# daviidsilvaa/MPI-Model

Measured on AMD Instinct MI355X. Metric: cell-updates/s (GCUPS) per step + % of HBM roofline, higher is better.
Workload: dtype f64; 1 GPU; c3: 32768x32768 fp64 global, row slabs (BASELINE configs[2]); ranks=1, rows_per_gpu=32768, n_attr=1, parallelism=row-slab x1, rows_per_wave=1656

## Files before the change

mpi-model_amd/csrc/mm_engine.hip:

```cpp
#include <rccl/rccl.h>

#include <algorithm>
#include <cmath>
#include <cstdio>
#include <cstdlib>
#include <cstring>
#include <map>
#include <string>
#include <vector>

#include "../../include/mpimodel.h"
#include "mm_inst.hpp"
#include "mm_plan.hpp"

static_assert(MM_FIELD_MAX_STEPS == mm::kFieldMaxSteps, "include/mpimodel.h: MM_FIELD_MAX_STEPS");

namespace {

thread_local std::string g_last_error;

int fail(int code, const std::string& msg) {
    g_last_error = msg;
    return code;
}
// ... 15 lines not shown
#define MM_TRY(expr)             \
    do {                         \
        int rc_ = (expr);        \
        if (rc_ != MM_OK) return rc_; \
    } while (0)

struct Transfer {
    int a, b;
    double rate;
};

struct Pass {
    std::vector<Transfer> pre, post;
    int diffuse_mask = 0;
    double drate[mm::kMaxAttr] = {0, 0, 0, 0};
    int field_mask = 0;
};

struct FlowDesc {
    int kind, a, b;
    double rate;
};

}

struct mm_engine {
    mm_desc d{};
    int na = 1;
    long long pitch = 0;
    long long rows_alloc = 0;
    double* base = nullptr;
    size_t bytes = 0;
    double* buf[2][mm::kMaxAttr] = {};
    int cur = 0;
    double* fld_base[mm::kMaxAttr] = {};
    double* fld[mm::kMaxAttr] = {};
    long long fld_rows[mm::kMaxAttr][2] = {};
    hipStream_t s_comp = nullptr, s_comm = nullptr;
    hipEvent_t ev_ready = nullptr, ev_halo = nullptr;
    hipEvent_t ev_comp_mark = nullptr, ev_comm_done = nullptr;
    bool comm_live = false;
    ncclComm_t comm = nullptr;

    std::vector<FlowDesc> flows;
    std::vector<Pass> passes;

    mm::PlanIn pin;
    int th_env = 8;
    std::map<const mm::KernelInst*, int> slots;
    bool self_halo = false;
    int variant = 0;
    double* partials = nullptr;
    long long partials_cap = 0;
    double* hist = nullptr;
    unsigned long long* hist_n = nullptr;
    long long hist_cap = 0;
    long long hist_host = 0;
    double* sum_tmp = nullptr;
    long long sum_blocks = 0;

    long long steps_done = 0;

    std::map<std::tuple<int, long long, long long, long long>, std::pair<hipGraphExec_t, int>> graphs;

    int graph_state = 0;
    long long graph_launches = 0;
    int graph_count = 0;
    std::string graph_note;

    bool timing = false;
    std::vector<hipEvent_t> ev_pool;
    std::vector<double> ev_bytes;
    size_t ev_used = 0;
    long long timed_launches = 0;
    double timed_ms = 0.0;
    double timed_bytes = 0.0;
};

namespace {

int set_device(mm_engine* e) {
    MM_HIP(hipSetDevice(e->d.device));
    return MM_OK;
}

void drop_graphs(mm_engine* e) {
    for (auto& kv : e->graphs) (void)hipGraphExecDestroy(kv.second.first);
    e->graphs.clear();
}

int compile_passes(mm_engine* e) {
    e->passes.clear();
    Pass cur;
    bool open = false;
    for (const FlowDesc& f : e->flows) {
        const bool fieldf = f.kind == MM_FLOW_DIFFUSE_FIELD;
        if (open && (fieldf ? (!cur.field_mask || (cur.field_mask & (1 << f.a))) : cur.field_mask != 0)) {
            e->passes.push_back(cur);
            open = false;
        }
        if (fieldf) {
            if (!open) {
                cur = Pass();
                open = true;
            }
            cur.field_mask |= 1 << f.a;
// ... 186 lines not shown
    return MM_OK;
}

int split_comm(mm_engine* e, int depth) {
    if (!e->comm_live) MM_HIP(hipStreamWaitEvent(e->s_comm, e->ev_comp_mark, 0));
    if (rccl_halo(e)) MM_TRY(halo_rccl(e, depth));
    MM_HIP(hipStreamWaitEvent(e->s_comm, e->ev_comp_mark, 0));
    return MM_OK;
}

int unsplit_halo(mm_engine* e, int depth) {
    if (!rccl_halo(e)) return MM_OK;
    MM_HIP(hipEventRecord(e->ev_ready, e->s_comp));
    MM_HIP(hipStreamWaitEvent(e->s_comm, e->ev_ready, 0));
    MM_TRY(halo_rccl(e, depth));
    MM_HIP(hipEventRecord(e->ev_halo, e->s_comm));
    MM_HIP(hipStreamWaitEvent(e->s_comp, e->ev_halo, 0));
    return MM_OK;
}

int launch(mm_engine* e, const mm::PassLaunches& pl, bool red, const mm::PassArgs& A, hipStream_t s,
           bool border) {
    const int nt = border ? 0 : e->variant;
    if (pl.kern.kernel != mm::kOneStep)
        MM_HIP(mm::launch_kstep(
            inst_key(e, pl.kern.kernel, pl.depth, pl.kern.cols, A.seg != 0, red, nt & 1), A, s));
    else if (A.field_mask)
        MM_HIP(mm::launch_field(e->na, red, A, s, nt));
    else
        MM_HIP(mm::launch_pass(e->na, red, A, s, e->variant));
    return MM_OK;
}

void set_launch(mm::PassArgs& A, const mm::Launch& l) {
    A.ra0 = (int)l.lo, A.ra1 = (int)l.hi, A.rb0 = (int)l.lo2, A.rb1 = (int)l.hi2;
    A.seg = l.seg, A.th = l.th, A.th_edge = l.th_edge, A.xcd_remap = l.xcd_remap;
    A.nstrips = l.nstrips;
    A.waves_a = l.waves_a, A.waves_total = l.waves_total, A.partial_base = l.partial_base;
    const mm::Wide6& w = l.c6;
    A.c6_top = w.top, A.c6_bot = w.bot, A.c6_col = w.col, A.c6_rcol = w.rcol;
    A.c6_strips = w.strips, A.c6_rstrips = w.rstrips, A.c6_th = w.th;
    A.c6_band0 = w.band0, A.c6_band1 = w.band1, A.c6_frame = w.frame;
}

int enqueue_pass(mm_engine* e, const Pass& p, int k, int mask, bool time_it, bool prime = false) {
    const bool red = mask != 0;
    const mm::PassLaunches pl = mm::pass_launches(e->pin, k, red);
    mm::PassArgs A;
    fill_args(e, p, A);
    const int perm = pl.kern.kernel == mm::kWide ? relabel(e, A) : kPermIdentity;
    mm::PassArgs B = A;
    set_launch(A, pl.interior);
    set_launch(B, pl.border);
    if (prime) {
        A.waves_total = B.waves_total = 0;
        A.waves_a = B.waves_a = -1;
        MM_TRY(launch(e, pl, red, A, e->s_comp, false));
        if (pl.split) MM_TRY(launch(e, pl, red, B, e->s_comm, true));
        return MM_OK;
    }
    if (pl.split)
        MM_TRY(split_comp(e));
    else if (e->pin.split)
        MM_TRY(unsplit_halo(e, pl.depth));
    hipEvent_t t0 = nullptr, t1 = nullptr;
    if (time_it) {
        t0 = next_event(e);
        t1 = next_event(e);
        if (!t0 || !t1) return fail(MM_ERR_HIP, "hipEventCreate failed");
        e->ev_bytes.resize(e->ev_used / 2);
        e->ev_bytes.back() = (16.0 * e->na + 8.0 * __builtin_popcount((unsigned)p.field_mask)) *
                             (double)(pl.interior.hi - pl.interior.lo) * (double)e->d.W;
        MM_HIP(hipEventRecord(t0, e->s_comp));
    }
    MM_TRY(launch(e, pl, red, A, e->s_comp, false));
    if (time_it) MM_HIP(hipEventRecord(t1, e->s_comp));
    if (pl.split) {
        MM_TRY(split_comm(e, pl.depth));
        MM_TRY(launch(e, pl, red, B, e->s_comm, true));
        MM_HIP(hipEventRecord(e->ev_comm_done, e->s_comm));
        e->comm_live = true;
        if (red) MM_HIP(hipStreamWaitEvent(e->s_comp, e->ev_comm_done, 0));
    }
    if (red && pl.kern.kernel == mm::kOneStep)
        MM_HIP(mm::launch_finalize(e->partials, pl.total, e->na, e->hist, e->hist_n, e->hist_cap,
                                   e->s_comp, 1));
    else if (red)
        MM_HIP(mm::launch_finalize_levels(e->partials, pl.total, k, e->na, mask, e->hist,
                                          e->hist_n, e->hist_cap, e->s_comp, perm));
    e->cur ^= 1;
    return MM_OK;
}

int enqueue_steps(mm_engine* e, long long first, long long n, long long reduce_every,
                  bool time_it) {
    long long s = first;
    const long long end = first + n;
    auto red = [&](long long step) { return reduce_every > 0 && step % reduce_every == 0; };
    if (mm::kstep_ok(e->pin)) {
        for (int k : mm::pass_lengths(e->pin, n)) {
            int mask = 0;
            for (int j = 0; j < k; ++j)
                if (red(s + j)) mask |= 1 << j;
            MM_TRY(enqueue_pass(e, e->passes[0], k, mask, time_it));
            s += k;
        }
    } else {
        const int np = (int)e->passes.size();
        for (; s < end; ++s)
            for (int pi = 0; pi < np; ++pi)
                MM_TRY(enqueue_pass(e, e->passes[pi], 1, red(s) && pi == np - 1, time_it));
    }
    if (e->comm_live) {
        MM_HIP(hipStreamWaitEvent(e->s_comp, e->ev_comm_done, 0));
        e->comm_live = false;
    }
    return MM_OK;
}

int agree_capture(mm_engine* e, bool ok) {
    if (!e->comm || e->d.nranks <= 1) return ok ? MM_OK : MM_ERR_HIP;
    int v = ok ? 1 : 0;
    int* dv = reinterpret_cast<int*>(e->sum_tmp);
    if (hipStreamSynchronize(e->s_comp) != hipSuccess ||
        hipStreamSynchronize(e->s_comm) != hipSuccess ||
        hipMemcpy(dv, &v, sizeof v, hipMemcpyHostToDevice) != hipSuccess ||
        ncclAllReduce(dv, dv, 1, ncclInt32, ncclMin, e->comm, e->s_comm) != ncclSuccess ||
// ... 176 lines not shown
        return fail(MM_ERR_INVALID, "mm_engine_create: a single slab must own the whole grid");
    if (d.halo_mode == MM_HALO_RCCL && !d.comm_id)
        return fail(MM_ERR_INVALID, "mm_engine_create: MM_HALO_RCCL needs comm_id");
    if (d.nranks > 1 && d.halo_mode == MM_HALO_NONE)
        return fail(MM_ERR_INVALID, "mm_engine_create: nranks > 1 needs a halo mode");
    if (d.W > (1LL << 30) || d.h > (1LL << 30))
        return fail(MM_ERR_INVALID, "mm_engine_create: slab too large");

    mm_engine* e = new mm_engine();
    e->d = d;
    e->na = d.n_attr;
    e->pitch = (d.W + mm::kStripCols - 1) / mm::kStripCols * mm::kStripCols;
    e->rows_alloc = d.h + 2 * mm::kGhost;
    mm::PlanIn& pin = e->pin;
    pin.H = d.H, pin.W = d.W, pin.h = d.h, pin.x_init = d.x_init, pin.nranks = d.nranks;
    pin.pitch = e->pitch, pin.n_attr = d.n_attr;
    pin.min_rows = std::min<long long>(d.h, d.H / d.nranks);
    pin.knobs = mm::read_knobs([](const char* name) -> const char* { return std::getenv(name); });
    e->th_env = pin.knobs.th;
    pin.slots = [e](mm::Kernel kernel, int k, bool red) { return slots_per_cu(e, kernel, k, red); };
    pin.slots6 = [e](int k) { return slots_per_cu(e, mm::kWide, k, false, mm::kWide6Cols); };
    e->variant = mm::kernel_variant(pin);

    auto cleanup = [&](int rc) {
        mm_engine_destroy(e);
        return rc;
    };
    hipError_t he = hipSetDevice(d.device);
    if (he != hipSuccess) return cleanup(fail(MM_ERR_HIP, std::string("hipSetDevice: ") + hipGetErrorString(he)));
    he = hipDeviceGetAttribute(&e->pin.ncu, hipDeviceAttributeMultiprocessorCount, d.device);
    if (he != hipSuccess || e->pin.ncu <= 0) e->pin.ncu = 256;

    const size_t per = (size_t)e->rows_alloc * (size_t)e->pitch;
    const size_t per_al = (per + 31) / 32 * 32;
    e->bytes = sizeof(double) * per_al * 2 * (size_t)e->na;
    if (hipStreamCreateWithFlags(&e->s_comp, hipStreamNonBlocking) != hipSuccess ||
        hipStreamCreateWithFlags(&e->s_comm, hipStreamNonBlocking) != hipSuccess ||
        hipEventCreateWithFlags(&e->ev_ready, hipEventDisableTiming) != hipSuccess ||
        hipEventCreateWithFlags(&e->ev_halo, hipEventDisableTiming) != hipSuccess ||
        hipEventCreateWithFlags(&e->ev_comp_mark, hipEventDisableTiming) != hipSuccess ||
        hipEventCreateWithFlags(&e->ev_comm_done, hipEventDisableTiming) != hipSuccess)
        return cleanup(fail(MM_ERR_HIP, "stream/event creation failed"));

    he = hipMalloc(&e->base, e->bytes);
    if (he != hipSuccess) return cleanup(fail(MM_ERR_NOMEM, std::string("hipMalloc: ") + hipGetErrorString(he)));
    he = hipMemsetAsync(e->base, 0, e->bytes, e->s_comp);
    if (he != hipSuccess) return cleanup(fail(MM_ERR_HIP, std::string("hipMemsetAsync: ") + hipGetErrorString(he)));
    for (int k = 0; k < 2; ++k)
        for (int a = 0; a < e->na; ++a)
            e->buf[k][a] = e->base + per_al * (size_t)(k * e->na + a) + mm::kGhost * e->pitch;

    int rc = ensure_partials(e);
    if (rc != MM_OK) return cleanup(rc);
    e->hist_cap = 1 << 12;
    if (hipMalloc(&e->hist, sizeof(double) * (size_t)e->hist_cap * e->na) != hipSuccess ||
        hipMalloc(&e->hist_n, 2 * sizeof(unsigned long long)) != hipSuccess ||
        hipMemsetAsync(e->hist_n, 0, 2 * sizeof(unsigned long long), e->s_comp) != hipSuccess)
        return cleanup(fail(MM_ERR_NOMEM, "history allocation failed"));
    e->sum_blocks = std::min<long long>(1024, std::max<long long>(1, d.h));
    if (hipMalloc(&e->sum_tmp, sizeof(double) * (size_t)(e->sum_blocks + mm::kMaxAttr)) != hipSuccess)
        return cleanup(fail(MM_ERR_NOMEM, "sum scratch allocation failed"));
    he = hipStreamSynchronize(e->s_comp);
    if (he != hipSuccess) return cleanup(fail(MM_ERR_HIP, std::string("hipStreamSynchronize: ") + hipGetErrorString(he)));

    e->self_halo = e->pin.knobs.self_halo && d.nranks == 1 && d.halo_mode == MM_HALO_RCCL;
    if ((d.nranks > 1 || e->self_halo) && d.halo_mode == MM_HALO_RCCL) {
        int v = 0;
        if (ncclGetVersion(&v) != ncclSuccess || v != NCCL_VERSION_CODE) {
            char msg[160];
            std::snprintf(msg, sizeof msg,
                          "RCCL %d loaded, engine built against %d: load libmpimodel_hip.so "
                          "before any library that bundles its own librccl (e.g. torch)",
                          v, NCCL_VERSION_CODE);
            return cleanup(fail(MM_ERR_RCCL, msg));
        }
        ncclUniqueId id;
        std::memcpy(&id, d.comm_id, sizeof id);
        ncclResult_t nr = ncclCommInitRank(&e->comm, d.nranks, id, d.rank);
        if (nr != ncclSuccess)
            return cleanup(fail(MM_ERR_RCCL, std::string("ncclCommInitRank: ") + ncclGetErrorString(nr)));
        long long hmin = d.h;
        double* dv = e->sum_tmp;
        if (hipMemcpy(dv, &hmin, sizeof hmin, hipMemcpyHostToDevice) != hipSuccess ||
            ncclAllReduce(dv, dv, 1, ncclInt64, ncclMin, e->comm, e->s_comm) != ncclSuccess ||
            hipStreamSynchronize(e->s_comm) != hipSuccess ||
            hipMemcpy(&hmin, dv, sizeof hmin, hipMemcpyDeviceToHost) != hipSuccess)
            return cleanup(fail(MM_ERR_RCCL, "min slab rows all-reduce failed"));
        e->pin.min_rows = hmin;
        e->pin.split = true;
    } else if (d.nranks > 1 && d.halo_mode == MM_HALO_HOST) {
        long long x0 = 0, hh = 0;
        if (mm_partition_rows(d.H, d.nranks, d.rank, &x0, &hh) != MM_OK || x0 != d.x_init ||
            hh != d.h)
            return cleanup(fail(MM_ERR_INVALID, "mm_engine_create: MM_HALO_HOST slabs must be "
                                                "mm_partition_rows(H, nranks, rank)"));
        e->pin.split = true;
    }
    *out = e;
    return MM_OK;
}

int mm_engine_destroy(mm_engine* e) {
    if (!e) return MM_OK;
    (void)hipSetDevice(e->d.device);
    if (e->s_comp) (void)hipStreamSynchronize(e->s_comp);
    if (e->s_comm) (void)hipStreamSynchronize(e->s_comm);
    drop_graphs(e);
    if (e->comm) (void)ncclCommDestroy(e->comm);
    for (hipEvent_t ev : e->ev_pool) (void)hipEventDestroy(ev);
    if (e->ev_ready) (void)hipEventDestroy(e->ev_ready);
    if (e->ev_halo) (void)hipEventDestroy(e->ev_halo);
    if (e->ev_comp_mark) (void)hipEventDestroy(e->ev_comp_mark);
    if (e->ev_comm_done) (void)hipEventDestroy(e->ev_comm_done);
    if (e->s_comp) (void)hipStreamDestroy(e->s_comp);
    if (e->s_comm) (void)hipStreamDestroy(e->s_comm);
    if (e->base) (void)hipFree(e->base);
    for (double* f : e->fld_base)
        if (f) (void)hipFree(f);
    if (e->partials) (void)hipFree(e->partials);
    if (e->hist) (void)hipFree(e->hist);
    if (e->hist_n) (void)hipFree(e->hist_n);
    if (e->sum_tmp) (void)hipFree(e->sum_tmp);
    (void)hipGetLastError();
    delete e;
    return MM_OK;
}

int mm_engine_info(mm_engine* e, mm_info* info) {
    if (!e || !info) return fail(MM_ERR_INVALID, "mm_engine_info: null");
    std::memset(info, 0, sizeof *info);
    info->pitch = e->pitch;
    info->bytes_device = (long long)e->bytes;
    info->n_passes = (int)e->passes.size();
    const mm::SlabPlan sp = mm::slab_plan(e->pin);
    info->kernel = sp.kernel;
    info->rows_per_wave = sp.rows_per_wave;
    info->waves_per_pass = sp.waves_per_pass;
    info->seg_waves_per_cu = sp.seg_waves_per_cu;
    if (sp.kernel == mm::kWide && e->na > 1)
        info->chain_kernel = (wring(e) && sp.steps_per_launch == 8) ? MM_CHAIN_RING : MM_CHAIN_RUNTIME;
    info->steps_done = e->steps_done;
    info->fused_attrs = e->na;
    info->steps_per_launch = info->halo_depth = sp.steps_per_launch;
    info->graph_state = e->graph_state;
    info->graph_count = e->graph_count;
    info->graph_launches = e->graph_launches;
    info->hist_entries = e->hist_host;
    std::snprintf(info->graph_note, sizeof info->graph_note, "%s", e->graph_note.c_str());
    return MM_OK;
}

int mm_fill(mm_engine* e, int attr, int mode, double value, unsigned long long seed) {
    if (!e || attr < 0 || attr >= e->na || (mode != MM_FILL_UNIFORM && mode != MM_FILL_RANDOM))
        return fail(MM_ERR_INVALID, "mm_fill: bad arguments");
    MM_TRY(set_device(e));
    MM_HIP(mm::launch_fill(e->buf[e->cur][attr], e->pitch, e->d.H, e->d.W, e->d.x_init, e->d.h,
                           mode, value, seed, e->s_comp));
    MM_HIP(hipStreamSynchronize(e->s_comp));
    e->steps_done = 0;
    return MM_OK;
}

int mm_upload(mm_engine* e, int attr, const double* host) {
    if (!e || !host || attr < 0 || attr >= e->na) return fail(MM_ERR_INVALID, "mm_upload: bad arguments");
    MM_TRY(set_device(e));
    MM_HIP(hipMemcpy2DAsync(e->buf[e->cur][attr], sizeof(double) * e->pitch, host,
                            sizeof(double) * e->d.W, sizeof(double) * e->d.W, e->d.h,
                            hipMemcpyHostToDevice, e->s_comp));
    MM_HIP(hipStreamSynchronize(e->s_comp));
    e->steps_done = 0;
    return MM_OK;
}
// ... 443 lines not shown
```

mpi-model_amd/csrc/mm_geom.hpp:

```cpp
#pragma once

namespace mm {

constexpr int kMaxAttr = 4;
constexpr int kMaxChain = 4;
constexpr int kStripCols = 128;
constexpr int kWavesPerBlock = 4;
constexpr int kBlock = 64 * kWavesPerBlock;
constexpr int kMaxSteps = 10;
constexpr int kMaxWide = 20;
constexpr int kGhost = kMaxWide;
constexpr int kBorderRows = 4;
constexpr int kSegPrefetch1 = 8;
constexpr int kWide20Waves = 4;
constexpr int kWideRingWaves = 4;
constexpr int kWide6Cols = 6;

constexpr int span3(long long n, long long i) {
    return (i >= 0 && i < n) ? 1 + (i > 0) + (i < n - 1) : 0;
}

inline int passk_out_cols(int k) { return kStripCols - 4 * ((k + 1) / 2); }

inline int passk_max_steps(int na) { return na == 1 ? kMaxSteps : 2; }

inline long long passk_max_rows(int k, long long pitch) {
    return (1LL << 31) / (pitch * 8) - (3 * k + 2 * kSegPrefetch1 + 8);
}

constexpr int kFieldMaxSteps = 4;
constexpr int kFieldPrefetch = 8;
constexpr int field_ring(int k) {
    return (kFieldPrefetch + 2 * (k - 1) + kFieldPrefetch - 1) / kFieldPrefetch * kFieldPrefetch;
}

inline long long fieldk_max_rows(int k, long long pitch) {
    return (1LL << 31) / (pitch * 8) - (3 * k + 2 * field_ring(k) + 8);
}

inline bool wide_has(int k, int c, int na) {
    if (na > 1) return na == 4 && c == 2 && (k == 4 || k == 8);
    return c == 4 && (k == 4 || k == 8 || k == 12 || k == 16 || k == 20);
}

inline int wide_out_cols(int k, int c) {
    return 64 * c - 2 * c * ((k + c - 1) / c);
}

struct Wide6Cols {
    int col, rcol, strips, rstrips;
};
inline Wide6Cols wide6_cols(long long W) {
    const int o4 = wide_out_cols(kMaxWide, 4), o6 = wide_out_cols(kMaxWide, kWide6Cols);
    const int halo = kWide6Cols * ((kMaxWide + kWide6Cols - 1) / kWide6Cols);
    const long long room = W - o4 - (halo + 1);
    const int n = room >= o6 && W < (1LL << 30) ? (int)(room / o6) : 0;
    const int rcol = o4 + n * o6;
    return {o4, rcol, n, n ? (int)((W - rcol + o4 - 1) / o4) : 0};
}

inline int wide_waves_per_block(int k, int c, int na, bool ring) {
    if (!wide_has(k, c, na)) return 0;
    if (na > 1 && k == 8 && ring) return kWideRingWaves;
    if (na == 1 && k == 20) return kWide20Waves;
    return 4;
}

}
```

mpi-model_amd/csrc/mm_internal.hpp:

```cpp
#pragma once

#include <hip/hip_runtime.h>

#include "mm_geom.hpp"

namespace mm {

struct PassArgs {
    const double* in[kMaxAttr];
    double* out[kMaxAttr];
    long long H, W, x_init, pitch;
    int ra0, ra1, rb0, rb1;
    int th;
    int nstrips;
    long long waves_a;
    long long waves_total;
    int diffuse_mask;
    int npre, npost;
    double drate[kMaxAttr];
    signed char pre_a[kMaxChain], pre_b[kMaxChain];
    signed char post_a[kMaxChain], post_b[kMaxChain];
    double pre_r[kMaxChain], post_r[kMaxChain];
    double* partials;
    long long partial_base;
    int xcd_remap;
    int seg;
    int th_edge;
    const double* field[kMaxAttr];
    int field_mask;
    int c6_top, c6_bot;
    int c6_col, c6_rcol;
    int c6_strips, c6_rstrips;
    int c6_th;
    long long c6_band0, c6_band1, c6_frame;
};

hipError_t launch_pass(int na, bool reduce, const PassArgs& a, hipStream_t s, int variant);
hipError_t launch_field(int na, bool reduce, const PassArgs& a, hipStream_t s, int variant);
hipError_t launch_finalize_levels(const double* partials, long long n, int k, int na, int mask,
                                  double* hist, unsigned long long* hist_n, long long cap,
                                  hipStream_t s, int perm);
hipError_t launch_fill(double* buf, long long pitch, long long H, long long W, long long x_init,
                       long long h, int mode, double value, unsigned long long seed, hipStream_t s);
hipError_t launch_point(double* buf, long long pitch, long long H, long long W, long long x_init,
                        long long h, long long sx, long long sy, double captured, double rate,
                        hipStream_t s);
hipError_t launch_finalize(const double* partials, long long n, int na, double* hist,
                           unsigned long long* hist_n, long long cap, hipStream_t s,
                           int entries = 1);
hipError_t launch_slab_sum(const double* buf, long long pitch, long long W, long long h,
                           double* partials, long long nblocks, double* out_sum, hipStream_t s);

}
```

mpi-model_amd/csrc/mm_plan.cpp:

```cpp
#include "mm_plan.hpp"

#include <algorithm>
#include <cmath>
#include <cstdlib>

namespace mm {

namespace {

constexpr double kAny = 1e300;

struct KnobRow {
    const char* name;
    char type;
    double lo, hi;
    void (*set)(Knobs&, double);
};

const KnobRow kKnobRows[] = {
    {"MM_GRAPH", 'i', -kAny, kAny, [](Knobs& k, double v) { k.graphs_ok = v != 0; }},
    {"MM_GRAPH_MIN_STEPS", 'i', 1, 256, [](Knobs& k, double v) { k.graph_min = (long long)v; }},
    {"MM_GRAPH_MAX_LAUNCHES", 'i', 1, 4096, [](Knobs& k, double v) { k.graph_max = (long long)v; }},
    {"MM_ROWS_PER_WAVE", 'i', 8, 32, [](Knobs& k, double v) { if (v == 8 || v == 16 || v == 32) k.th = (int)v; }},
    {"MM_FUSE", 'i', -kAny, kAny, [](Knobs& k, double v) { k.passk = k.passk && v != 0; }},
    {"MM_PASSK", 'i', -kAny, kAny, [](Knobs& k, double v) { k.passk = k.passk && v != 0; }},
    {"MM_WIDE", 'i', -kAny, kAny, [](Knobs& k, double v) { k.wide = v != 0 ? 1 : 0; }},
    {"MM_STEPS_PER_PASS", 'i', 1, kAny,
     [](Knobs& k, double d) {
         const int v = (int)std::min(d, 1e9);
         if (v <= kMaxSteps || (k.wide != 0 && (wide_has(v, 4, 1) || wide_has(v, 2, 4)))) k.kpass = v;
         k.kpass_multi = std::min(v, 2);
     }},
    {"MM_PASS_PLAN", 'i', -kAny, kAny, [](Knobs& k, double v) { k.plan = v != 0; }},
    {"MM_SEG_WAVES", 'd', 0, kAny, [](Knobs& k, double v) { k.seg_waves = v; }},
    {"MM_SEG_EDGE", 'd', 0, 1, [](Knobs& k, double v) { k.seg_edge = v; }},
    {"MM_XCD_REMAP", 'i', -kAny, kAny, [](Knobs& k, double v) { k.xcd = v != 0; }},
    {"MM_BORDER_SEGMENTS", 'i', -kAny, kAny, [](Knobs& k, double v) { k.border_segments = v != 0; }},
    {"MM_CHAIN_RING", 'i', -kAny, kAny, [](Knobs& k, double v) { k.ring_ok = v != 0; }},
    {"MM_SYNC_SPIN", 'i', -kAny, kAny, [](Knobs& k, double v) { k.sync_spin = v != 0; }},
    {"MM_SELF_HALO", 'i', -kAny, kAny, [](Knobs& k, double v) { k.self_halo = v != 0; }},
    {"MM_KERNEL_VARIANT", 'i', 0, kAny, [](Knobs& k, double v) { k.variant = (int)std::min(v, 1e9); }},
    {"MM_FIELD_STEPS", 'i', 0, kFieldMaxSteps, [](Knobs& k, double v) { k.field_steps = (int)v; }},
    {"MM_FIELD_HALO", 'i', 1, kFieldMaxSteps, [](Knobs& k, double v) { k.field_halo = (int)v; }},
    {"MM_WIDE_COLS", 'i', 4, kWide6Cols, [](Knobs& k, double v) { if (v != 5) k.wide_cols = (int)v; }},
};

}

Knobs read_knobs(const std::function<const char*(const char*)>& get) {
    Knobs k;
    for (const KnobRow& r : kKnobRows) {
        const char* s = get(r.name);
        if (!s) continue;
        const double v = r.type == 'i' ? (double)std::atoll(s) : std::atof(s);
        if ((r.type == 'i' ? v >= r.lo : v > r.lo) && v <= r.hi) r.set(k, v);
    }
    return k;
}

namespace {

constexpr double kWideCells = 268435456.0;
constexpr double kWideSmallCells = 33554432.0;
constexpr int kWideSmallAuto = 8;
constexpr double kWideSplitCells = 134217728.0;
constexpr int kWideAuto = 20;
constexpr int kWideAutoMulti = 8;

double slab_cells(const PlanIn& in) { return (double)in.min_rows * (double)in.W; }

int wcols(const PlanIn& in) { return in.n_attr > 1 ? 2 : 4; }

bool wide_big(const PlanIn& in) {
    return in.knobs.wide > 0 || slab_cells(in) >= kWideCells ||
           (in.knobs.wide < 0 && in.n_attr == 1 && slab_cells(in) >= kWideSplitCells);
}

bool wide_on(const PlanIn& in) {
    return in.knobs.wide > 0 ||
           (in.knobs.wide < 0 && (in.n_attr > 1 || wide_big(in) || slab_cells(in) < kWideSmallCells));
}

bool use_wide(const PlanIn& in, int k) {
    return wide_on(in) && passk_ok(in) && wide_has(k, wcols(in), in.n_attr) &&
           (in.n_attr == 1 || in.diffuse_mask != 0);
}

long long ceil_div(long long a, long long b) { return (a + b - 1) / b; }

int passk_steps(const PlanIn& in) {
    const Knobs& kn = in.knobs;
    const bool wide1 = wide_on(in) && in.n_attr == 1;
    const int kauto = wide1 ? (wide_big(in) ? kWideAuto : kWideSmallAuto)
                            : (slab_cells(in) >= kWideSplitCells ? 8 : 7);
    int k1 = kn.kpass > 0 ? kn.kpass : kauto;
    if (!wide1) k1 = std::min(k1, kMaxSteps);
    int k = in.n_attr == 1 ? k1 : std::min(kn.kpass_multi, passk_max_steps(in.n_attr));
// ... 359 lines not shown
```

mpi-model_amd/csrc/mm_plan.hpp:

```cpp
#pragma once

#include <functional>
#include <vector>

#include "mm_geom.hpp"

namespace mm {

struct Knobs {
    bool graphs_ok = true;
    long long graph_min = 16;
    long long graph_max = 128;
    int th = 8;
    bool passk = true;
    int wide = -1;
    int kpass = 0;
    int kpass_multi = 2;
    bool plan = true;
    double seg_waves = 0.0;
    double seg_edge = 0.0;
    bool border_segments = true;
    int xcd = 0;
    bool ring_ok = true;
    bool sync_spin = true;
    bool self_halo = false;
    int variant = -1;
    int field_steps = 0;
    int field_halo = 1;
    int wide_cols = 0;
};
Knobs read_knobs(const std::function<const char*(const char*)>& get);

enum Kernel { kOneStep = 0, kPassK = 2, kWide = 3, kFieldK = 4 };

struct PlanIn {
    long long H = 0, W = 0, h = 0, x_init = 0;
    int nranks = 1;
    long long min_rows = 0;
    long long pitch = 0;
    int n_attr = 1;
    bool split = false;
    int n_passes = 0;
    int diffuse_mask = 0;
    bool chains = false;
    bool ring = false;
    bool field = false;
    int field_k = 0;
    Knobs knobs;
    int ncu = 0;
    std::function<int(Kernel, int k, bool red)> slots;
    std::function<int(int k)> slots6;
};

struct KernelChoice {
    Kernel kernel;
    int cols;
    long long strips;
};

struct Segments {
    int th, th_edge;
    long long count;
};

struct Wide6 {
    int top = 0, bot = 0, col = 0, rcol = 0, strips = 0, rstrips = 0, th = 0;
    long long band0 = 0, band1 = 0, frame = 0;
};

struct Launch {
    long long lo = 0, hi = 0, lo2 = 0, hi2 = 0;
    int seg = 0, th = 0, th_edge = 0, xcd_remap = 0, nstrips = 0;
    long long waves_a = 0, waves_total = 0, partial_base = 0;
    Wide6 c6;
};

struct PassLaunches {
    KernelChoice kern;
    int depth;
    bool split;
    Launch interior, border;
    long long total;
// ... 28 lines not shown
```

mpi-model_amd/csrc/mm_wide.hpp:

```cpp
#pragma once

#include "mm_passk.hpp"

#ifndef MM_WIDE_GEN_ROW
#define MM_WIDE_GEN_ROW 1
#endif

namespace mm {

namespace {

#ifndef MM_WIDE_U
#define MM_WIDE_U 4
#endif
#ifndef MM_WIDE_B
#define MM_WIDE_B 4
#endif
#ifndef MM_WIDE_MIN_WAVES
#define MM_WIDE_MIN_WAVES 2
#endif
#ifndef MM_WIDE_PRO_MID
#define MM_WIDE_PRO_MID 1
#endif
#ifndef MM_WIDE_ASC
// ... 373 lines not shown
                const dv2 v = src[64 * (a * H2 + h) + x.lane];
                cur[a][2 * h] = v.x;
                cur[a][2 * h + 1] = v.y;
            }
        }
    }
    if (!PRO) t = i - x.start;
    double uin[NA][C];
#pragma unroll
    for (int a = 0; a < NA; ++a) {
#pragma unroll
        for (int k = 0; k < C; ++k) uin[a][k] = cur[a][k];
    }
#pragma unroll
    for (int qq = 0; qq < KW; ++qq) {
        const int q = kSkew == 2 ? qq : KW - 1 - qq;
        const int m = t - kSkew * q;
        if (PRO && m < 0) continue;
        const int j = x.p * KW + q + 1;
        const long long gx = x.g0 + (j - 1) + m;
        double u[NA][C];
#pragma unroll
        for (int a = 0; a < NA; ++a) {
#pragma unroll
            for (int k = 0; k < C; ++k)
                u[a][k] = kSkew == 2 ? cur[a][k] : (q == 0 ? uin[a][k] : st.pend[q - 1][a][k]);
        }
        const int e1 = (PK + q + 1) & 1;
        const int e = (PK + q + 1 + tp - kSkew * q) & 1;
        if (PRO && m < 2) {
            lfill<C, NA, BODY>(x, gx, m, e1, st.win[q], u);
            continue;
        }
        double o[NA][C];
        lemit<C, NA, BODY>(x, gx, e, st.win[q], u, o);
        if (RED) {
            if constexpr (OWNED) {
#pragma unroll
                for (int a = 0; a < NA; ++a) {
#pragma unroll
                    for (int k = 0; k < C; ++k)
                        st.acc[q][a] = __builtin_fma(o[a][k], x.c.ownw[k], st.acc[q][a]);
                    asm volatile("" : "+v"(st.acc[q][a]));
                }
            } else {
                const int r = x.rA - K + m + j - 2;
#pragma unroll
                for (int a = 0; a < NA; ++a) accumc<C>(st.acc[q][a], r >= x.oA && r < x.rB, x.c, o[a]);
            }
        }
        if (q == KW - 1) {
            if (kOut) {
                const int ro = m - 2 - (x.oA - x.rA);
                const unsigned so = x.soff + (unsigned)(ro < 0 ? 0 : ro) * x.rowb;
#pragma unroll
                for (int a = 0; a < NA; ++a) {
                    const __amdgpu_buffer_rsrc_t rs = ro < 0 ? x.none : x.out[a];
#pragma unroll
                    for (int h = 0; h < H2; ++h)
                        store_row<NT>(rs, so + 16 * h, o[a][2 * h], o[a][2 * h + 1]);
                }
            } else {
                dv2* dst = x.lds_out + (i % G::RL) * RW;
#pragma unroll
                for (int a = 0; a < NA; ++a) {
#pragma unroll
                    for (int h = 0; h < H2; ++h) {
                        dv2 v;
                        v.x = o[a][2 * h];
                        v.y = o[a][2 * h + 1];
                        dst[64 * (a * H2 + h) + x.lane] = v;
                    }
                }
            }
        } else {
#pragma unroll
            for (int a = 0; a < NA; ++a) {
#pragma unroll
                for (int k = 0; k < C; ++k) {
                    if (kSkew == 2)
                        cur[a][k] = o[a][k];
                    else
                        st.pend[q][a][k] = o[a][k];
                }
            }
        }
    }
}

template <int P, int B>
__device__ __forceinline__ void group_end(int i) {
    if (P > 1 && (i + 1) % B == 0) wg_sync();
}

template <int C, int NA, int KW, int P, int U, int B, bool RED, int NT, int BODY, int ROLE,
          int PP, bool OWNED = false>
__device__ __forceinline__ void wave_groups(const WCtx<C, NA>& x, WState<C, NA, KW, U>& st,
                                            int b0, int b1) {
    static_assert(B % 2 == 0, "row pairs: an even number of iterations per group");
    constexpr int PD = (PP * WGeom<KW, P, B>::D) & 1;
    for (int base = b0; base < b1; base += B) {
#pragma unroll
        for (int tt = 0; tt < B; ++tt)
            wave_iter<C, NA, KW, P, U, B, RED, NT, BODY, ROLE, false, PP, OWNED>(
                x, st, base + tt, 0, tt % U, (tt + PD) & 1);
        if (P > 1) wg_sync();
    }
}

template <int C, int NA, int KW, int P, int U, int B, bool RED, int NT, int ROLE, int BODY,
// ... 182 lines not shown
        }
    }
    const int need = (P - 1) * G::D + G::S0 + (x.rB - x.rA);
    const int iend = (need + G::B - 1) / G::B * G::B;
    const bool hasL = c0 < 1, hasR = c0 + 64 * C - 1 >= W - 1;
    x.c.eL = hasL && y0 == 0;
    x.c.eR = hasR && y0 + C - 1 == W - 1;
    x.c.gen = (hasL && hasR) || (hasR && (W - 1 - c0) % C != C - 1);
    if (!hasL && !hasR)
        wave_dispatch<C, NA, KW, P, U, B, RED, NT, kBodyFast>(x, iend, carry);
    else
        wave_dispatch<C, NA, KW, P, U, B, RED, NT, kBodyEdge>(x, iend, carry);
}

template <int C, int NA, int KW, int P, int MW, int U, int B, bool RED, int NT>
__global__ __launch_bounds__(64 * P, MW) void mm_wide_kernel(const PassArgs A) {
    using G = WGeom<KW, P, B>;
    constexpr int K = G::K;
    constexpr int RW = 32 * C * NA;
    __shared__ dv2 lds[(P > 1 ? P - 1 : 1) * G::RL * RW];
    const int lane = threadIdx.x & 63;
    const int p = __builtin_amdgcn_readfirstlane(threadIdx.x >> 6);
    const long long blk = blockIdx.x;
    if (blk >= A.waves_total) return;
    int rlo, rhi;
    long long w = blk;
    if (w < A.waves_a) {
        rlo = A.ra0;
        rhi = A.ra1;
    } else {
        w -= A.waves_a;
        rlo = A.rb0;
        rhi = A.rb1;
    }
    int strip, rA, rB;
    seg_map(w, rlo, rhi, A.nstrips, A.th, A.th_edge, strip, rA, rB);
    double carry[KW][NA];
#pragma unroll
    for (int q = 0; q < KW; ++q) {
#pragma unroll
        for (int a = 0; a < NA; ++a) carry[q][a] = 0.0;
    }
    wide_segment<C, NA, KW, P, U, B, RED, NT>(A, lds, p, lane, strip, rA, rB, carry);
    if (RED && lane == 0) {
#pragma unroll
        for (int q = 0; q < KW; ++q) {
#pragma unroll
            for (int a = 0; a < NA; ++a)
                A.partials[((A.partial_base + blk) * K + p * KW + q) * NA + a] = carry[q][a];
        }
    }
}

template <int C, int KW, int P, int U, int B, int NT, int ROLE, int PP>
__device__ __forceinline__ void wave_run_fast(const WCtx<C, 1>& x, int iend) {
    static_assert(B % U == 0, "ring slots repeat within a group");
    WState<C, 1, KW, U> st;
    const int s = wave_prologue<C, 1, KW, P, U, B, false, NT, ROLE, kBodyFast, PP>(x, st);
    wave_groups<C, 1, KW, P, U, B, false, NT, kBodyFast, ROLE, PP>(x, st, s, iend);
}

template <int C, int KW, int P, int U, int B, int NT>
__device__ __forceinline__ void fast_segment(const PassArgs& A, dv2* lds, int p, int lane,
                                             long long col, int rA, int rB) {
    using G = WGeom<KW, P, B>;
    constexpr int K = G::K;
    constexpr int LH = (K + C - 1) / C;
    constexpr int RW = 32 * C;
    WCtx<C, 1> x;
    const int sh = (int)((A.x_init + rA - K) & 1);
    x.rA = rA - sh;
    x.oA = rA;
    x.rB = rB;
    const long long y0 = col - C * LH + C * lane;
    const bool in_row = y0 >= 0 && y0 + C <= A.pitch;
    const bool store_lane = lane >= LH && lane < 64 - LH && y0 + C <= A.W;
    x.rowb = (unsigned)(A.pitch * 8);
    x.voff = (in_row ? (unsigned)(y0 * 8) : kOOB) - (unsigned)sh * x.rowb;
    x.soff = store_lane ? (unsigned)(y0 * 8) : kOOB;
    x.c.H = A.H;
    x.p = p;
    x.lane = lane;
    x.start = p * G::D;
    x.dmask = 1;
    x.g0 = A.x_init + x.rA - K;
    x.r8[0] = A.drate[0] * 0.125;
    x.in[0] = rows_rsrc(A.in[0] + (long long)(rA - K) * A.pitch, rB - rA + 2 * K, A.pitch);
    x.out[0] = rows_rsrc(A.out[0] + (long long)rA * A.pitch, rB - rA, A.pitch);
    x.none = rows_rsrc(A.out[0], 0, A.pitch);
    x.lds_in = p > 0 ? lds + (p - 1) * G::RL * RW : lds;
    x.lds_out = p < P - 1 ? lds + p * G::RL * RW : lds;
    x.A = &A;
    const int need = (P - 1) * G::D + G::S0 + (x.rB - x.rA);
    const int iend = (need + G::B - 1) / G::B * G::B;
    constexpr bool kMidPar = ((KW | G::D) & 1) != 0;
    if (p == 0)
        wave_run_fast<C, KW, P, U, B, NT, kRoleFirst, 0>(x, iend);
    else if (p == P - 1)
        wave_run_fast<C, KW, P, U, B, NT, kRoleLast, (P - 1) & 1>(x, iend);
    else if (kMidPar && (p & 1))
        wave_run_fast<C, KW, P, U, B, NT, kRoleMid, 1>(x, iend);
    else
        wave_run_fast<C, KW, P, U, B, NT, kRoleMid, 0>(x, iend);
}

template <int CF, int CI, int KW, int P, int MW, int U, int B, int NT>
__global__ __launch_bounds__(64 * P, MW) void mm_wide6_kernel(const PassArgs A) {
    using G = WGeom<KW, P, B>;
    constexpr int K = G::K;
    constexpr int LHI = (K + CI - 1) / CI;
    constexpr int OCI = 64 * CI - 2 * CI * LHI;
    static_assert(CI >= CF && CI % 2 == 0 && OCI % 2 == 0, "the LDS rows hold either path's");
    __shared__ dv2 lds[(P - 1) * G::RL * 32 * CI];
    const int lane = threadIdx.x & 63;
    const int p = __builtin_amdgcn_readfirstlane(threadIdx.x >> 6);
    long long w = blockIdx.x;
    if (w >= A.waves_total) return;
    int strip, rA, rB;
    if (w >= A.c6_frame) {
        seg_map(w - A.c6_frame, A.c6_top, A.c6_bot, A.c6_strips, A.c6_th, A.c6_th, strip, rA, rB);
        fast_segment<CI, KW, P, U, B, NT>(A, lds, p, lane, A.c6_col + (long long)strip * OCI, rA,
                                          rB);
        return;
    }
    double carry[KW][1];
    long long col0 = 0;
    if (w < A.c6_band0) {
        seg_map(w, A.ra0, A.c6_top, A.nstrips, A.c6_top - A.ra0, A.c6_top - A.ra0, strip, rA, rB);
    } else if (w < A.c6_band1) {
        seg_map(w - A.c6_band0, A.c6_bot, A.ra1, A.nstrips, A.ra1 - A.c6_bot, A.ra1 - A.c6_bot,
                strip, rA, rB);
    } else {
        seg_map(w - A.c6_band1, A.c6_top, A.c6_bot, 1 + A.c6_rstrips, A.th, A.th, strip, rA, rB);
        if (strip > 0) {
            col0 = A.c6_rcol;
            strip -= 1;
        }
    }
    wide_segment<CF, 1, KW, P, U, B, false, NT>(A, lds, p, lane, strip, rA, rB, carry, col0);
}

template <int C, int NA, int KW, int P>
bool wide_key(const InstKey& q) {
    return q.family == kInstWide && q.k == KW * P && q.cols == C && q.na == NA && q.seg;
}

template <int C, int NA, int KW, int P, int MW, bool RED, int NT>
const KernelInst* wide_inst_v() {
    return inst_of<mm_wide_kernel<C, NA, KW, P, MW, MM_WIDE_U, MM_WIDE_B, RED, NT>, 64 * P>();
}

template <int C, int NA, int KW, int P, int MW>
const KernelInst* wide_inst(const InstKey& q) {
    if (!wide_key<C, NA, KW, P>(q)) return nullptr;
    if (q.nt)
        return q.red ? wide_inst_v<C, NA, KW, P, MW, true, 1>()
                     : wide_inst_v<C, NA, KW, P, MW, false, 1>();
    return q.red ? wide_inst_v<C, NA, KW, P, MW, true, 0>()
                 : wide_inst_v<C, NA, KW, P, MW, false, 0>();
}

}

}
```

Baseline: 3580 GCUPS.

## Add optional chained row-block claiming for wide6 fast-path workgroups

Adds a chaining mode in which a wide6 fast-path workgroup, as it nears the end of its row block, atomically claims the next row block in the same strip. If the claim succeeds it carries on in place, keeping its pipeline warm instead of paying another prologue. Per-strip claim words are allocated and zeroed before each pass, and new knobs select the mode and run length. With the default settings chaining is off, but the block-to-segment ordering still changes (edge strips first, then first and last row blocks), and the wave loop becomes a phase loop. Risks are extra atomics and memset work, and changed load balance when chaining is enabled.

```diff
diff --git a/mpi-model_amd/csrc/mm_engine.hip b/mpi-model_amd/csrc/mm_engine.hip
--- a/mpi-model_amd/csrc/mm_engine.hip
+++ b/mpi-model_amd/csrc/mm_engine.hip
@@ -91,6 +91,8 @@
     int variant = 0;
     double* partials = nullptr;
     long long partials_cap = 0;
+    int* claims = nullptr;
+    long long claims_cap = 0;
     double* hist = nullptr;
     unsigned long long* hist_n = nullptr;
     long long hist_cap = 0;
@@ -383,6 +385,15 @@
     mm::PassArgs B = A;
     set_launch(A, pl.interior);
     set_launch(B, pl.border);
+    long long nclaims = 0;
+    if (A.c6_strips > 0 && A.c6_bot > A.c6_top) {
+        A.c6_chain = mm::chain_mode(e->pin.knobs.wide6_chain, A.c6_th, A.pitch);
+        A.c6_run = e->pin.knobs.wide6_run;
+        A.c6_claims = e->claims;
+        if (A.c6_chain != mm::kChainOff)
+            nclaims = (long long)A.c6_strips * ((A.c6_bot - A.c6_top + A.c6_th - 1) / A.c6_th);
+        if (nclaims > e->claims_cap) return fail(MM_ERR_INVALID, "claim words: plan beyond the allocation");
+    }
     if (prime) {
         A.waves_total = B.waves_total = 0;
         A.waves_a = B.waves_a = -1;
@@ -404,6 +415,7 @@
                              (double)(pl.interior.hi - pl.interior.lo) * (double)e->d.W;
         MM_HIP(hipEventRecord(t0, e->s_comp));
     }
+    if (nclaims) MM_HIP(hipMemsetAsync(e->claims, 0, sizeof(int) * (size_t)nclaims, e->s_comp));
     MM_TRY(launch(e, pl, red, A, e->s_comp, false));
     if (time_it) MM_HIP(hipEventRecord(t1, e->s_comp));
     if (pl.split) {
@@ -686,6 +698,11 @@
 
     int rc = ensure_partials(e);
     if (rc != MM_OK) return cleanup(rc);
+    if (e->na == 1 && mm::wide6_cols(d.W).strips > 0) {
+        e->claims_cap = (long long)mm::wide6_cols(d.W).strips * (d.h / 16 + 1);
+        if (hipMalloc(&e->claims, sizeof(int) * (size_t)e->claims_cap) != hipSuccess)
+            return cleanup(fail(MM_ERR_NOMEM, "claim words allocation failed"));
+    }
     e->hist_cap = 1 << 12;
     if (hipMalloc(&e->hist, sizeof(double) * (size_t)e->hist_cap * e->na) != hipSuccess ||
         hipMalloc(&e->hist_n, 2 * sizeof(unsigned long long)) != hipSuccess ||
@@ -752,6 +769,7 @@
     for (double* f : e->fld_base)
         if (f) (void)hipFree(f);
     if (e->partials) (void)hipFree(e->partials);
+    if (e->claims) (void)hipFree(e->claims);
     if (e->hist) (void)hipFree(e->hist);
     if (e->hist_n) (void)hipFree(e->hist_n);
     if (e->sum_tmp) (void)hipFree(e->sum_tmp);
diff --git a/mpi-model_amd/csrc/mm_geom.hpp b/mpi-model_amd/csrc/mm_geom.hpp
--- a/mpi-model_amd/csrc/mm_geom.hpp
+++ b/mpi-model_amd/csrc/mm_geom.hpp
@@ -59,6 +59,69 @@
     return {o4, rcol, n, n ? (int)((W - rcol + o4 - 1) / o4) : 0};
 }
 
+constexpr int kWide6Group = 4;
+constexpr int kWide6Prefetch = 2;
+constexpr int kWide6Fill = 52;
+
+enum { kChainOff = 0, kChainOn = 1, kChainHeads = 2 };
+
+constexpr int chain_answer_iter(int rows) {
+    return (rows + 2 * kMaxWide - kWide6Prefetch) / kWide6Group * kWide6Group;
+}
+constexpr int chain_claim_iter(int rows) { return chain_answer_iter(rows) - kWide6Group; }
+
+constexpr int kChainMinRows =
+    (kWide6Fill + kWide6Group - 1) / kWide6Group * kWide6Group + kWide6Group -
+    (2 * kMaxWide - kWide6Prefetch);
+static_assert(chain_claim_iter(kChainMinRows) >= kWide6Fill &&
+                  chain_claim_iter(kChainMinRows - 1) < (kWide6Fill + 3) / 4 * 4,
+              "the attempt follows every wave's prologue");
+
+constexpr bool chain_fits(int th, long long pitch) {
+    return (long long)(th + 2 * kMaxWide) * pitch * 8 < (1LL << 31);
+}
+
+constexpr int chain_mode(int mode, int th, long long pitch) {
+    return (mode == kChainOn || mode == kChainHeads) && th >= kChainMinRows && chain_fits(th, pitch)
+               ? mode
+               : kChainOff;
+}
+constexpr int chain_run(int run, int per) { return run < 1 ? 1 : (run > per ? per : run); }
+constexpr bool chain_block_starts(int mode, int rb, int run, int per) {
+    return mode != kChainHeads || rb % chain_run(run, per) == 0;
+}
+constexpr bool chain_tries_next(int mode, int rb, int run, int per) {
+    return mode != kChainOff && rb + 1 < per &&
+           (mode != kChainHeads || (rb + 1) % chain_run(run, per) != 0);
+}
+
+struct SegStart {
+    int strip, rb;
+};
+
+constexpr SegStart seg_start_plain(long long t, int ns, int per) {
+    if (ns < 3) return {(int)(t % ns), (int)(t / ns)};
+    if (t < 2LL * per) return {t < per ? 0 : ns - 1, (int)(t % per)};
+    const long long u = t - 2LL * per;
+    const int q = (int)(u / (ns - 2));
+    return {1 + (int)(u % (ns - 2)), q == 0 ? 0 : (q == 1 ? per - 1 : q - 1)};
+}
+
+constexpr SegStart chain_start(long long t, int ns, int per, int run) {
+    const int G = chain_run(run, per);
+    if (G == 1) return seg_start_plain(t, ns, per);
+    const int strip = (int)(t % ns);
+    int q = (int)(t / ns);
+    const int a = per / G, b = per % G;
+    const int heads = a + (b > 0);
+    if (q < heads) return {strip, q * G};
+    q -= heads;
+    const int hi = G - (b > 1 ? b : 1);
+    if (q < hi * a) return {strip, (q % a) * G + (G - 1 - q / a)};
+    q -= hi * a;
+    return {strip, (q % (a + 1)) * G + (b - 1 - q / (a + 1))};
+}
+
 inline int wide_waves_per_block(int k, int c, int na, bool ring) {
     if (!wide_has(k, c, na)) return 0;
     if (na > 1 && k == 8 && ring) return kWideRingWaves;
diff --git a/mpi-model_amd/csrc/mm_internal.hpp b/mpi-model_amd/csrc/mm_internal.hpp
--- a/mpi-model_amd/csrc/mm_internal.hpp
+++ b/mpi-model_amd/csrc/mm_internal.hpp
@@ -33,6 +33,8 @@
     int c6_strips, c6_rstrips;
     int c6_th;
     long long c6_band0, c6_band1, c6_frame;
+    int* c6_claims;
+    int c6_chain, c6_run;
 };
 
 hipError_t launch_pass(int na, bool reduce, const PassArgs& a, hipStream_t s, int variant);
diff --git a/mpi-model_amd/csrc/mm_plan.cpp b/mpi-model_amd/csrc/mm_plan.cpp
--- a/mpi-model_amd/csrc/mm_plan.cpp
+++ b/mpi-model_amd/csrc/mm_plan.cpp
@@ -43,6 +43,8 @@
     {"MM_FIELD_STEPS", 'i', 0, kFieldMaxSteps, [](Knobs& k, double v) { k.field_steps = (int)v; }},
     {"MM_FIELD_HALO", 'i', 1, kFieldMaxSteps, [](Knobs& k, double v) { k.field_halo = (int)v; }},
     {"MM_WIDE_COLS", 'i', 4, kWide6Cols, [](Knobs& k, double v) { if (v != 5) k.wide_cols = (int)v; }},
+    {"MM_WIDE6_CHAIN", 'i', kChainOff, kChainHeads, [](Knobs& k, double v) { k.wide6_chain = (int)v; }},
+    {"MM_WIDE6_RUN", 'i', 1, kAny, [](Knobs& k, double v) { k.wide6_run = (int)std::min(v, 1e9); }},
 };
 
 }
diff --git a/mpi-model_amd/csrc/mm_plan.hpp b/mpi-model_amd/csrc/mm_plan.hpp
--- a/mpi-model_amd/csrc/mm_plan.hpp
+++ b/mpi-model_amd/csrc/mm_plan.hpp
@@ -28,6 +28,8 @@
     int field_steps = 0;
     int field_halo = 1;
     int wide_cols = 0;
+    int wide6_chain = kChainOff;
+    int wide6_run = 4;
 };
 Knobs read_knobs(const std::function<const char*(const char*)>& get);
 
diff --git a/mpi-model_amd/csrc/mm_wide.hpp b/mpi-model_amd/csrc/mm_wide.hpp
--- a/mpi-model_amd/csrc/mm_wide.hpp
+++ b/mpi-model_amd/csrc/mm_wide.hpp
@@ -449,10 +449,11 @@
         if (q == KW - 1) {
             if (kOut) {
                 const int ro = m - 2 - (x.oA - x.rA);
-                const unsigned so = x.soff + (unsigned)(ro < 0 ? 0 : ro) * x.rowb;
+                constexpr bool kWrapDrop = C == kWide6Cols && BODY == kBodyFast && NA == 1 && !RED;
+                const unsigned so = x.soff + (unsigned)(ro < 0 && !kWrapDrop ? 0 : ro) * x.rowb;
 #pragma unroll
                 for (int a = 0; a < NA; ++a) {
-                    const __amdgpu_buffer_rsrc_t rs = ro < 0 ? x.none : x.out[a];
+                    const __amdgpu_buffer_rsrc_t rs = ro < 0 && !kWrapDrop ? x.none : x.out[a];
 #pragma unroll
                     for (int h = 0; h < H2; ++h)
                         store_row<NT>(rs, so + 16 * h, o[a][2 * h], o[a][2 * h + 1]);
@@ -741,17 +742,96 @@
     }
 }
 
+
+__device__ __forceinline__ int chain_claim(int* word) {
+    int seen = 0;
+    __hip_atomic_compare_exchange_strong(word, &seen, 1, __ATOMIC_RELAXED, __ATOMIC_RELAXED,
+                                         __HIP_MEMORY_SCOPE_AGENT);
+    return seen;
+}
+
+__device__ __forceinline__ __amdgpu_buffer_rsrc_t rows_rsrc_uniform(const double* first, int rows,
+                                                                    long long pitch) {
+    const unsigned long long a = (unsigned long long)first;
+    const unsigned lo = __builtin_amdgcn_readfirstlane((unsigned)a);
+    const unsigned hi = __builtin_amdgcn_readfirstlane((unsigned)(a >> 32));
+    const int bytes = __builtin_amdgcn_readfirstlane(rows > 0 ? (int)(rows * pitch * 8) : 0);
+    return __builtin_amdgcn_make_buffer_rsrc(
+        reinterpret_cast<double*>(((unsigned long long)hi << 32) | lo), 0, bytes, 0x00020000);
+}
+
+struct FastRun {
+    int* claims;
+    volatile int* word;
+    int rb, per;
+    int th, bot;
+    int mode, run;
+};
+
+enum { kRunToClaim = 0, kRunToAnswer = 1, kRunToEnd = 2 };
+
 template <int C, int KW, int P, int U, int B, int NT, int ROLE, int PP>
-__device__ __forceinline__ void wave_run_fast(const WCtx<C, 1>& x, int iend) {
+__device__ __forceinline__ void wave_run_fast(WCtx<C, 1>& x, const PassArgs& A, FastRun r) {
+    using G = WGeom<KW, P, B>;
+    constexpr int K = G::K;
+    constexpr int kFill = (P - 1) * G::D + G::S0;
     static_assert(B % U == 0, "ring slots repeat within a group");
+    static_assert(kFill == kWide6Fill && B == kWide6Group && U == kWide6Prefetch && K == kMaxWide,
+                  "mm_geom.hpp: the chained schedule's constants");
     WState<C, 1, KW, U> st;
-    const int s = wave_prologue<C, 1, KW, P, U, B, false, NT, ROLE, kBodyFast, PP>(x, st);
-    wave_groups<C, 1, KW, P, U, B, false, NT, kBodyFast, ROLE, PP>(x, st, s, iend);
+    int base = wave_prologue<C, 1, KW, P, U, B, false, NT, ROLE, kBodyFast, PP>(x, st);
+    int rows = x.rB - x.rA;
+    int ibase = x.oA - K, obase = x.oA;
+    int phase = chain_tries_next(r.mode, r.rb, r.run, r.per) ? kRunToClaim : kRunToEnd;
+    for (;;) {
+        rows = __builtin_amdgcn_readfirstlane(rows);
+        phase = __builtin_amdgcn_readfirstlane(phase);
+        ibase = __builtin_amdgcn_readfirstlane(ibase);
+        obase = __builtin_amdgcn_readfirstlane(obase);
+        if (ROLE == kRoleFirst)
+            x.in[0] = rows_rsrc_uniform(A.in[0] + (long long)ibase * A.pitch, x.rB + K - ibase, A.pitch);
+        if (ROLE == kRoleLast)
+            x.out[0] = rows_rsrc_uniform(A.out[0] + (long long)obase * A.pitch, x.rB - obase, A.pitch);
+        const int ans = chain_answer_iter(rows);
+        const int stop = phase == kRunToClaim    ? ans - B
+                         : phase == kRunToAnswer ? ans
+                                                 : (kFill + rows + B - 1) / B * B;
+        const int b0 = __builtin_amdgcn_readfirstlane(base);
+        const int b1 = __builtin_amdgcn_readfirstlane(stop);
+        __builtin_assume(b0 >= 0 && b0 % B == 0);
+        wave_groups<C, 1, KW, P, U, B, false, NT, kBodyFast, ROLE, PP>(x, st, b0, b1);
+        base = b1;
+        if (phase == kRunToEnd) break;
+        if (phase == kRunToClaim) {
+            if (ROLE == kRoleFirst && x.lane == 0) *r.word = chain_claim(r.claims + r.rb + 1);
+            phase = kRunToAnswer;
+            continue;
+        }
+        if (__builtin_amdgcn_readfirstlane(*r.word) != 0) {
+            phase = kRunToEnd;
+            continue;
+        }
+        r.rb = __builtin_amdgcn_readfirstlane(r.rb + 1);
+        const int nrB = __builtin_amdgcn_readfirstlane(min(x.rB + r.th, r.bot));
+        if (ROLE == kRoleFirst) {
+            const int nb = x.rA - K + base;
+            x.voff -= (unsigned)(nb - ibase) * x.rowb;
+            ibase = nb;
+        }
+        if (ROLE == kRoleLast) {
+            const int nb = x.rA + base - kFill;
+            x.soff -= (unsigned)(nb - obase) * x.rowb;
+            obase = nb;
+        }
+        rows += nrB - x.rB;
+        x.rB = nrB;
+        phase = chain_tries_next(r.mode, r.rb, r.run, r.per) ? kRunToClaim : kRunToEnd;
+    }
 }
 
 template <int C, int KW, int P, int U, int B, int NT>
 __device__ __forceinline__ void fast_segment(const PassArgs& A, dv2* lds, int p, int lane,
-                                             long long col, int rA, int rB) {
+                                             long long col, int rA, int rB, const FastRun& r) {
     using G = WGeom<KW, P, B>;
     constexpr int K = G::K;
     constexpr int LH = (K + C - 1) / C;
@@ -780,17 +860,15 @@
     x.lds_in = p > 0 ? lds + (p - 1) * G::RL * RW : lds;
     x.lds_out = p < P - 1 ? lds + p * G::RL * RW : lds;
     x.A = &A;
-    const int need = (P - 1) * G::D + G::S0 + (x.rB - x.rA);
-    const int iend = (need + G::B - 1) / G::B * G::B;
     constexpr bool kMidPar = ((KW | G::D) & 1) != 0;
     if (p == 0)
-        wave_run_fast<C, KW, P, U, B, NT, kRoleFirst, 0>(x, iend);
+        wave_run_fast<C, KW, P, U, B, NT, kRoleFirst, 0>(x, A, r);
     else if (p == P - 1)
-        wave_run_fast<C, KW, P, U, B, NT, kRoleLast, (P - 1) & 1>(x, iend);
+        wave_run_fast<C, KW, P, U, B, NT, kRoleLast, (P - 1) & 1>(x, A, r);
     else if (kMidPar && (p & 1))
-        wave_run_fast<C, KW, P, U, B, NT, kRoleMid, 1>(x, iend);
+        wave_run_fast<C, KW, P, U, B, NT, kRoleMid, 1>(x, A, r);
     else
-        wave_run_fast<C, KW, P, U, B, NT, kRoleMid, 0>(x, iend);
+        wave_run_fast<C, KW, P, U, B, NT, kRoleMid, 0>(x, A, r);
 }
 
 template <int CF, int CI, int KW, int P, int MW, int U, int B, int NT>
@@ -801,15 +879,31 @@
     constexpr int OCI = 64 * CI - 2 * CI * LHI;
     static_assert(CI >= CF && CI % 2 == 0 && OCI % 2 == 0, "the LDS rows hold either path's");
     __shared__ dv2 lds[(P - 1) * G::RL * 32 * CI];
+    __shared__ volatile int chain_word;
     const int lane = threadIdx.x & 63;
     const int p = __builtin_amdgcn_readfirstlane(threadIdx.x >> 6);
     long long w = blockIdx.x;
     if (w >= A.waves_total) return;
     int strip, rA, rB;
     if (w >= A.c6_frame) {
-        seg_map(w - A.c6_frame, A.c6_top, A.c6_bot, A.c6_strips, A.c6_th, A.c6_th, strip, rA, rB);
-        fast_segment<CI, KW, P, U, B, NT>(A, lds, p, lane, A.c6_col + (long long)strip * OCI, rA,
-                                          rB);
+        const int per = (A.c6_bot - A.c6_top + A.c6_th - 1) / A.c6_th;
+        const SegStart o = A.c6_chain ? chain_start(w - A.c6_frame, A.c6_strips, per, A.c6_run)
+                                      : seg_start_plain(w - A.c6_frame, A.c6_strips, per);
+        if (!chain_block_starts(A.c6_chain, o.rb, A.c6_run, per)) return;
+        FastRun r;
+        r.claims = A.c6_claims + (long long)o.strip * per;
+        r.word = &chain_word;
+        r.rb = o.rb, r.per = per, r.th = A.c6_th, r.bot = A.c6_bot;
+        r.mode = A.c6_chain, r.run = A.c6_run;
+        if (r.mode != kChainOff) {
+            if (threadIdx.x == 0) chain_word = chain_claim(r.claims + o.rb);
+            wg_sync();
+            if (__builtin_amdgcn_readfirstlane(chain_word) != 0) return;
+        }
+        rA = A.c6_top + o.rb * A.c6_th;
+        rB = min(rA + A.c6_th, A.c6_bot);
+        fast_segment<CI, KW, P, U, B, NT>(A, lds, p, lane, A.c6_col + (long long)o.strip * OCI, rA,
+                                          rB, r);
         return;
     }
     double carry[KW][1];
```

Result: no change. 3592 GCUPS, median of 2 (+0.4%).
